# zhoujun-7/VPHO

Measured on AMD Instinct MI355X. Metric: eval images/sec (bs=64, sample_num=100, steps=50); MPJPE delta vs ref, higher is better.
Workload: dtype f32; 1 GPU; vpho_net.forward(mode=predict), README eval config (BASELINE.json configs[1]); per_gpu_batch=64, sample_num=100, sampling_steps=50, topk_hand=30, topk_obj=10, crop=256x256, pipeline_depth=3, parallelism=dp1, score_mfma=f32, conv_mfma=f32, winograd_3x3=True

## Files before the change

### include/vpho_hip.h

```cpp
#ifndef VPHO_HIP_H
#define VPHO_HIP_H

#if defined(__GNUC__) || defined(__clang__)
#define VPHO_API __attribute__((visibility("default")))
#else
#define VPHO_API
#endif

#ifdef __cplusplus
extern "C" {
#endif

VPHO_API const char* vpho_last_error(void);
VPHO_API int vpho_abi_version(void);

VPHO_API int vpho_prof_enable(int kernel_class, int on);
VPHO_API int vpho_prof_collect(int kernel_class, double* total_ms, long long* launches, double* total_flops, double* total_bytes);

typedef struct {
    const float* x; const float* w; const float* bias;
    const float* in_scale; const float* in_shift;
    const float* res; float* y;
    int N, H, W, Cin, x_ld;
    int Cout, KH, KW, stride, pad_y, pad_x, OH, OW;
    long long y_sn, y_sy, y_sx;
    long long r_sn, r_sy, r_sx;
    float in_slope, out_slope;
    int w_ld, splits;
    long long x_split, w_split, y_split;
    const float* gate;
    float gate_slope;
    const int* row_map;
    const int* row_count;
    int rows_hint;
    int rows_scatter;
    const void* w_planes;
    int plane_terms;
    const float* res_up;
    int ru_H, ru_W, ru_ld;
    const float* x2;
    int Cin2, x2_ld, stride2, H2, W2;
    int groups;
    long long x_group, w_group, bias_group, y_group, res_group, x2_group, pre_group, ru_group;
    float* stats;
    int* stats_rows;
    int stats_cap;
    const float* bn_x; const float* bn_mean; const float* bn_invstd; const float* bn_gamma; const float* bn_beta;
} vpho_conv_desc;
VPHO_API int vpho_conv2d_nhwc_f32(const vpho_conv_desc* d, void* stream);
VPHO_API int vpho_conv3x3_winograd_nhwc_f32(const float* x, const float* u, const float* bias, int N, int H, int W, int Cin, int x_ld, int Cout,
                                   float out_slope, float* y, int y_ld, void* stream);
VPHO_API int vpho_conv3x3_winograd_grouped_nhwc_f32(const float* x, long long x_group, const float* u, const float* bias, int groups, int N, int H, int W,
                                           int Cin, int x_ld, int Cout, float out_slope, float* y, int y_ld, void* stream);
VPHO_API int vpho_winograd_window_tiles_i32(const int* wins, int N, int* tile_base, void* stream);
VPHO_API int vpho_conv3x3_winograd_scatter_nhwc_f32(const float* x, const float* u, const float* bias, int N, int H, int W, int Cin, int x_ld, int Cout,
                                           float out_slope, const int* wins, const int* tile_base, float* y, int y_ld, void* stream);
VPHO_API int vpho_winograd_weights_f32(const float* w_packed, int Cout, int Cin, int for_input_gradient, float* u, void* stream);
VPHO_API int vpho_winograd_weights_multi_f32(const void* segments, int n_segments, long long total_blocks, void* stream);
VPHO_API int vpho_conv3x3_winograd_gate_nhwc_f32(const float* x, const float* u, const float* gate, float gate_slope, int N, int H, int W, int Cin,
                                        int x_ld, int Cout, float* y, int y_ld, void* stream);
VPHO_API int vpho_conv3x3_winograd_stats_nhwc_f32(const float* x, const float* u, const float* bias, int N, int H, int W, int Cin, int x_ld, int Cout,
                                         float out_slope, float* y, int y_ld, float* stats, int stats_cap, int* stats_rows, const float* bn_x,
                                         const float* bn_mean, const float* bn_invstd, const float* bn_gamma, const float* bn_beta,
                                         float gate_slope, void* stream);
VPHO_API int vpho_conv3x3_winograd_rows_nhwc_f32(const float* x, const float* u, const float* bias, int N, int H, int W, int Cin, int x_ld, int Cout,
                                        float out_slope, const int* wins, const int* tile_base, int tiles_hint, float* y_rows, int y_ld,
                                        void* stream);

typedef struct {
    int D, Dp, nheads;
    const float *t_W, *t_w, *t_b, *pe0_w, *pe0_b, *pe2_w, *pe2_b, *w1_t, *w1_p, *w1_f, *b1, *w2, *b2;
    const void* w1_p_split;
    int split_terms;
} vpho_score_weights;

VPHO_API long long vpho_score_workspace_bytes(const vpho_score_weights* w, int bs, int S);

VPHO_API int vpho_score_eval(const vpho_score_weights* w, const float* feat_img, int bs, int S, const float* x, float t,
                    float* out, void* workspace, long long workspace_bytes, void* stream);

typedef struct {
    int nfev;
    int n_accepted, n_rejected;
    int nan_count;
    int status;
    int n_log;
} vpho_ode_stats;

VPHO_API int vpho_ode_sample(const vpho_score_weights* w, const float* feat_img, int bs, int S, const float* init_x,
                    double T0, double eps, int num_steps, double rtol, double atol,
                    void* xs_out, int xs_is_f64, void* x_out, int x_is_f64,
                    void* workspace, long long workspace_bytes,
                    vpho_ode_stats* stats_host, double* step_log_host, int step_log_cap, void* stream);

VPHO_API int vpho_nchw_to_nhwc_f32(const float* x, int N, int C, int H, int W, float* y, int ldy, void* stream);
VPHO_API int vpho_nhwc_to_nchw_f32(const float* x, int N, int H, int W, int C, int ldx, float* y, void* stream);
VPHO_API int vpho_maxpool_nhwc_f32(const float* x, int N, int H, int W, int C, int k, int stride, int pad, float* y, void* stream);
VPHO_API int vpho_resize_bilinear_nhwc_f32(const float* x, int N, int H, int W, int C, int ldx, int OH, int OW,
                                  float* y, int ldy, int c_off, int accumulate, void* stream);
VPHO_API int vpho_roi_align_nhwc_f32(const float* feat, int N, int H, int W, int C, const float* boxes, float spatial_scale,
                            int out_size, const unsigned char* flip_w, float* out, int ldo, int c_off, void* stream);
VPHO_API int vpho_roi_windows_i32(const float* boxes_a, const float* boxes_b, int N, int H, int W, float spatial_scale, int dilate,
                         int* wins, int* row_map, int* row_count, void* stream);
VPHO_API int vpho_resize_bilinear_rows_nhwc_f32(const float* x, int N, int H, int W, int C, int ldx, int OH, int OW, float* y, int ldy, int c_off,
                                       int accumulate, const int* row_map, const int* row_count, int rows_hint, void* stream);
VPHO_API int vpho_roi_align_window_nhwc_f32(const float* feat_rows, const int* wins, int N, int H, int W, int C, const float* boxes,
                                   float spatial_scale, int out_size, const unsigned char* flip_w, float* out, int ldo, int c_off, int rows_hint,
                                   void* stream);
VPHO_API int vpho_roi_align_window_dual_nhwc_f32(const float* feat_rows, const int* wins, int N, int H, int W, int C, const float* boxes,
                                        float spatial_scale, int out_size, const unsigned char* flip_w, float* out, int ldo, int c_off,
                                        const unsigned char* flip_w2, float* out2, int ldo2, int c_off2, int rows_hint, void* stream);
VPHO_API int vpho_align_heatmap_nhwc_f32(const float* hm, int N, int size, int C, const float* bbox, const float* bbox_rect,
                                const unsigned char* flip_w, float* out, void* stream);
VPHO_API int vpho_linear_acc64_f32(const float* x, int rows, int cin, int ld_x, const float* w, const float* bias, int cout, float out_slope,
                          float* y, int ld_y, void* stream);
VPHO_API int vpho_nerf_embed_f32(const float* g, int N, const unsigned char* flip_x, float* out, void* stream);
VPHO_API int vpho_cross_tokens_f32(const float* proj_hand, const float* proj_obj, const float* grav_emb, const float* pe,
                          int bs, float* out, void* stream);
VPHO_API int vpho_mha_f32(const float* qkv, int S, int B, int E, int nhead, float* out, void* stream);
VPHO_API int vpho_mha_dropout_f32(const float* qkv, int S, int B, int E, int nhead, const float* drop_mask, float* out, void* stream);
VPHO_API int vpho_add_layernorm_f32(const float* x, const float* r, const float* gamma, const float* beta, long long rows, int E,
                           float eps, float* out, void* stream);
VPHO_API int vpho_force_local_f32(const float* scale, int ld_scale, const float* logits, int ld_logits, const float* anchor,
                         float friction, long long rows, int group, int group_stride, int off_scale, int off_logits,
                         float* out, void* stream);
VPHO_API int vpho_rot6d_to_axis_angle_f32(const float* x, long long rows, int rot_per_row, int ldx, float* out, int ldo, void* stream);
VPHO_API int vpho_append_betas_f32(const float* betas, long long rows, long long rows_per_image, float* out, int ldo, void* stream);

typedef struct {
    const float *v_template;
    const float *shapedirs;
    const float *posedirs_t;
    const float *J_regressor;
    const float *weights;
    const float *tip_posedirs_t;
    const float *posedirs_mfma;
} vpho_mano_tables;
VPHO_API int vpho_mano_shape_f32(const vpho_mano_tables* t, const float* betas, int n_img, float* v_shaped, float* J, void* stream);
VPHO_API int vpho_mano_fk_f32(const vpho_mano_tables* t, const float* pose, int ld_pose, long long n_hands, int hands_per_image,
                     const float* v_shaped, const float* J, const unsigned char* ho3d_per_image,
                     float* verts, float* joints, void* stream);

typedef struct { const float* kpt; const float* vert; const float* com; int n_kpt, n_vert, n_obj; } vpho_obj_tables;
typedef struct { const int* face_idx; const float* anchor_weight; const float* vert2joint; const int* skeleton; } vpho_anchor_tables;

VPHO_API int vpho_hand_candidates_f32(const float* diff_pose, int ld_diff, const float* reg_pose, int bs, int S, float* pose, void* stream);
VPHO_API int vpho_hand_heat_f32(const float* joints, const float* root, const float* Kmat, const float* bbox, const float* heatmap,
                       int bs, int C, int J, int H, int W, const int* observe_host, int n_obs, float* out, void* stream);
VPHO_API int vpho_hand_fuse_level_f32(const float* hv, int n_obs, float* pose, int bs, int C, int k, int level,
                             float* val, int* idx, float* topk_pose, float* score_out, void* stream);
VPHO_API int vpho_topk_f32(const float* scores, int rows_outer, int n, int F, int k, float* val, int* idx, void* stream);
VPHO_API int vpho_topk_weights_f32(const float* val, int rows, int k, float* w, void* stream);
VPHO_API int vpho_obj_heat_score(const double* pose, int n, const double* transl_override, const float* root, const vpho_obj_tables* t,
                        const int* obj_id, const unsigned char* is_right, const float* Kmat, const float* bbox,
                        const float* heatmap, int bs, int H, int W, float* score, void* stream);
VPHO_API int vpho_obj_cross_candidates(const double* pose, int n, const int* transl_idx, const int* rot_idx, int bs, int ko, double* cand, void* stream);
VPHO_API int vpho_obj_physics_score(const double* cand, int n, const float* root, const vpho_obj_tables* t, const int* obj_id,
                           const unsigned char* is_right, const float* force_point, const float* force_global, int bs,
                           float* score, void* stream);
VPHO_API int vpho_obj_fuse_f64(const double* pose, int n, const int* idx_a, const float* w_a, const int* idx_b, const float* w_b,
                      const unsigned char* pick_b, int bs, int k, double* fused, void* stream);
VPHO_API int vpho_obj_verts_f32(const double* pose, const float* root, const vpho_obj_tables* t, const int* obj_id,
                       const unsigned char* is_right, int bs, float* out, void* stream);
VPHO_API int vpho_force_anchor_f32(const vpho_anchor_tables* t, const float* verts, const float* root, const float* force_local,
                          long long n_hands, int hands_per_image, float* force_point, float* force_global, void* stream);
VPHO_API int vpho_hand_phys_candidates_f32(const float* agg_pose, int ld_agg, const float* betas, const float* topk_pose, int bs, int k,
                                  float* out, void* stream);
VPHO_API int vpho_hand_phys_score_f32(const float* force_point, const float* force_global, const float* obj_vert, int n_vert,
                             int bs, int n_cand, float* finger_score, void* stream);
VPHO_API int vpho_hand_phys_fuse_f32(const float* cand, int n_cand, const int* idx, int bs, int k, float* out, void* stream);

VPHO_API int vpho_heatmap_peak_f32(const float* heatmap, long long n_maps, int H, int W, float* peak, int* ind, void* stream);
VPHO_API int vpho_hand_pt2d_score_f32(const float* joints, const float* root, const float* Kmat, const float* bbox, const float* peak,
                             int bs, int C, int per_joint, float* score, void* stream);
VPHO_API int vpho_obj_pt2d_score(const double* pose, int n, const float* root, const vpho_obj_tables* t, const int* obj_id,
                        const unsigned char* is_right, const float* Kmat, const float* bbox, const float* peak, int bs,
                        float* score, void* stream);
VPHO_API int vpho_hand_pose_fuse_f32(const float* pose, int ld_pose, int C, const int* idx, const float* w, int bs, int n, float* fused,
                            void* stream);
VPHO_API int vpho_hand_joint_gather_mean_f32(const float* joints, const int* idx, int bs, int C, int k, float* fused, void* stream);
// ... 198 lines not shown
```

### vpho_amd/model/engine.py

```python
import os

import torch

from .. import ops
from ..configs.args import cfg, AGGREGATION_MODES_HAND, AGGREGATION_MODES_OBJ
from . import pack as P

MANO_JOINT_LEVEL = {0: [0], 1: [1, 5, 9, 13, 17], 2: [2, 6, 10, 14, 18], 3: [3, 7, 11, 15, 19], 4: [4, 8, 12, 16, 20]}
PHY_TOPK = 5
DEFAULT_MODE = 'heatmap_cascade'


def _signature(model):
    import itertools
    v = p = 0
    for t in itertools.chain(model.parameters(), model.buffers()):
        v += t._version
        p ^= t.data_ptr()
    return v, p, str(next(model.parameters()).device)


def _stack2(a, b):
    if torch.is_tensor(a):
        return torch.stack([a, b]).contiguous()
# ... 25 lines not shown
            out = []
            for i in range(blocks):
                p = f'{fe}.{name}.0.{i}'
                blk = dict(c1=fold(p + '.conv1', p + '.bn1'), c2=fold(p + '.conv2', p + '.bn2'),
                           c3=fold(p + '.conv3', p + '.bn3'), stride=stride if i == 0 else 1, down=None)
                if (p + '.downsample.0.weight') in sd:
                    blk['down'] = fold(p + '.downsample.0', p + '.downsample.1')
                    blk['c3_down'] = (torch.cat([blk['c3'][0], blk['down'][0]], 1).contiguous(), (blk['c3'][1] + blk['down'][1]).contiguous())
                out.append(blk)
            return out

        self.layers = dict(layer1_h=res_layer('layer1_h', 3, 1), layer2_h=res_layer('layer2_h', 4, 2),
                           layer3_h=res_layer('layer3_h', 6, 2), layer4_h=res_layer('layer4_h', 3, 2),
                           layer2_o=res_layer('layer2_o', 4, 2), layer3_o=res_layer('layer3_o', 6, 2))
        self.fpn = {k: fold(f'{fe}.{k}') for k in ('toplayer_h', 'toplayer_o', 'smooth3_h', 'smooth3_o', 'latlayer1_h',
                                                   'latlayer2_h', 'latlayer3_h', 'latlayer1_o', 'latlayer2_o', 'latlayer3_o')}

        def hm_head(p):
            s, t = P.bn_affine(sd, p + '.deconv_layers.1')
            wd = sd[p + '.deconv_layers.0.weight'] * s[None, :, None, None]
            phases = {k: (d(w), py, px) for k, (w, py, px) in P.pack_deconv4x4s2(wd).items()}
            return dict(c0=fold(p + '.conv_layers.0'), c1=fold(p + '.conv_layers.1', p + '.conv_layers.2'), deconv=phases,
                        deconv_b=d(t), final=fold(p + '.final_layer'))

        self.hm = dict(hand=hm_head('head_hm_hand'), obj=hm_head('head_hm_obj'))

        def encoder(p, cin):
            cin_pad = (cin + 3) // 4 * 4
            blocks = []
            for i in range(8):
                q = f'{p}.reg.{i}'
                s, t = P.bn_affine(sd, q + '.bn')
                blocks.append(dict(pre=(d(s), d(t)), c1=fold(q + '.conv1', q + '.bn1'), c2=fold(q + '.conv2', q + '.bn2'), c3=fold(q + '.conv3')))
            return dict(project=fold(p + '.project', cin_pad=cin_pad), blocks=blocks, cin_pad=cin_pad)

        self.enc = dict(hand=encoder('encoder_hand', 277), obj=encoder('encoder_obj', 283))

        self.grouped = os.environ.get('VPHO_GROUPED', '1') != '0'
        self.head64 = os.environ.get('VPHO_HEAD_F64', '1') != '0'
        if self.grouped:
            L, F = self.layers, self.fpn
            self.g_layers = dict(layer2=_stack2(L['layer2_h'], L['layer2_o']), layer3=_stack2(L['layer3_h'], L['layer3_o']))
            self.g_fpn = {k: _stack2(F[k + '_h'], F[k + '_o']) for k in ('toplayer', 'latlayer1', 'latlayer2')}
            self.g_hm = _stack2(*({k: v for k, v in self.hm[s].items() if k != 'final'} for s in ('hand', 'obj')))
            self.g_enc = _stack2(encoder('encoder_hand', 283), self.enc['obj'])

        lin = lambda p: (d(sd[p + '.weight']), d(sd[p + '.bias']))
        self.head_mano = dict(l0=lin('head_mano.base_layer.0'), l2=lin('head_mano.base_layer.2'), pose=lin('head_mano.fc_pose'),
                              shape=lin('head_mano.fc_shape'))

        def cross(p):
            a = p + '.attn.layers.0'
            return dict(proj_hand=fold(p + '.proj_hand'), proj_obj=fold(p + '.proj_obj'),
                        grav=(d(torch.nn.functional.pad(sd[p + '.gravity_proj.weight'], (0, 1))), d(sd[p + '.gravity_proj.bias'])),
                        pe=d(sd[p + '.pose_embedder.pe'][:, 0, :]),
                        in_proj=(d(sd[a + '.self_attn.in_proj_weight']), d(sd[a + '.self_attn.in_proj_bias'])),
                        out_proj=lin(a + '.self_attn.out_proj'), l1=lin(a + '.linear1'), l2=lin(a + '.linear2'),
                        n1=lin(a + '.norm1'), n2=lin(a + '.norm2'))

        self.cross = dict(hand=cross('cross_hand'), obj=cross('cross_obj'))
        self.phys = dict(s0=lin('head_physics.fc_scale.0'), s2=lin('head_physics.fc_scale.2'), w0=lin('head_physics.fc_weight.0'),
                         w2=lin('head_physics.fc_weight.2'), anchor=d(sd['head_physics.anchor']))

        self.score_hand = ops.ScoreNet(sd, 'denoiser_hand', dev)
        self.score_obj = ops.ScoreNet(sd, 'denoiser_obj', dev)
        mano = dict(v_template=sd['head_mano.mano_layer.th_v_template'][0], shapedirs=sd['head_mano.mano_layer.th_shapedirs'],
                    posedirs=sd['head_mano.mano_layer.th_posedirs'], J_regressor=sd['head_mano.mano_layer.th_J_regressor'],
                    weights=sd['head_mano.mano_layer.th_weights'])
        self.mano = ops.Mano(mano, dev)
        names = model.head_obj.names
        ycb = {n: dict(kpt3d=sd[f'head_obj.point_{n}'], verts_sampled=sd[f'head_obj.vert_{n}'], CoM=sd[f'head_obj.CoM_{n}'][0]) for n in names}
        self.agg = ops.Aggregation(dict(ycb=ycb, anchor=model.assets['anchor']), model.anchor_skeleton, dev)
        self.last_info = {}
        self._obj_stream = None
        self._pin = {}
        from concurrent.futures import ThreadPoolExecutor
        self._obj_worker = ThreadPoolExecutor(max_workers=1, thread_name_prefix='vpho-obj-sampler')
        self.use_graphs = os.environ.get('VPHO_GRAPHS', '1') != '0'
        self.roi_window = os.environ.get('VPHO_ROI_WINDOW', '1') != '0'
        self.feature_streams = int(os.environ.get('VPHO_FEATURE_STREAMS', '1'))
        self.fpn_fuse = os.environ.get('VPHO_FPN_FUSE', '1') != '0'
        self.down_fuse = os.environ.get('VPHO_DOWN_FUSE', '1') != '0'
        self.winograd = os.environ.get('VPHO_WINOGRAD', '1') != '0'
        self.conv_terms = {'f32': 0, 'bf16x6': 6, 'bf16x9': 9}[os.environ.get('VPHO_CONV_MFMA', 'f32')]
        self.serial_samplers = False
        self.device_prior = os.environ.get('VPHO_DEVICE_PRIOR', '0') == '1'
        self.keep_states = False
        self._feat_side = None
        self._two_streams = False
        from .graphs import GraphedCall
        self._features_graph = GraphedCall(self.features, dev)
        self._aggregate_graph = GraphedCall(self._aggregate_from_tensors, dev)

    def stale(self, model):
        return _signature(model) != self.sig

    def _bottleneck(self, x, b, out=None, groups=1, x_shared=False):
        y = ops.conv2d_nhwc(x, *b['c1'], out_slope=0.01, groups=groups, x_shared=x_shared)
        if b['stride'] == 1:
            y = ops.conv3x3(y, *b['c2'], out_slope=0.01, winograd=self.winograd, groups=groups)
        else:
            y = ops.conv2d_nhwc(y, *b['c2'], kh=3, kw=3, stride=b['stride'], pad=1, out_slope=0.01, groups=groups)
        if b['down'] is not None and self.down_fuse and x.shape[-1] % 32 == 0 and y.shape[-1] % 32 == 0:
            return ops.conv2d_nhwc(y, *b['c3_down'], x2=x, stride2=b['stride'], out_slope=0.01, out=out, groups=groups, x2_shared=x_shared)
        r = x if b['down'] is None else ops.conv2d_nhwc(x, *b['down'], stride=b['stride'], groups=groups, x_shared=x_shared)
        return ops.conv2d_nhwc(y, *b['c3'], res=r, out_slope=0.01, out=out, groups=groups)

    def _layer(self, x, blocks, out=None, groups=1, x_shared=False):
        for i, b in enumerate(blocks):
            x = self._bottleneck(x, b, out if i == len(blocks) - 1 else None, groups, x_shared and i == 0)
        return x

    def _side(self):
        import contextlib
        if not self._two_streams:
            return contextlib.nullcontext()
        if self._feat_side is None:
            self._feat_side = torch.cuda.Stream(self.dev)
        self._feat_side.wait_stream(torch.cuda.current_stream())
        return torch.cuda.stream(self._feat_side)

    def _join(self):
        if self._two_streams:
            torch.cuda.current_stream().wait_stream(self._feat_side)

    def _stem(self, rgb):
        x = ops.nchw_to_nhwc(rgb, 4)
        c1 = ops.maxpool_nhwc(ops.conv2d_nhwc(x, *self.stem, kh=7, kw=7, stride=2, pad=3, out_slope=0.01), 3, 2, 1)
        return self._layer(c1, self.layers['layer1_h'])

    def _lateral(self, c, wb, p, rows=None, groups=1):
        if self.fpn_fuse:
            return ops.conv2d_nhwc(c, *wb, rows=rows, rows_scatter=rows is not None, res_up=p, groups=groups)
        q = ops.conv2d_nhwc(c, *wb, rows=rows, rows_scatter=rows is not None, groups=groups)
        return ops.resize_bilinear_nhwc(p, q.shape[1], q.shape[2], out=q, accumulate=True, rows=rows)

    def _top_down(self, fpn, sfx, c5, c4, c3, groups=1):
        p = ops.conv2d_nhwc(c5, *fpn['toplayer' + sfx], groups=groups)
        p = self._lateral(c4, fpn['latlayer1' + sfx], p, groups=groups)
        return self._lateral(c3, fpn['latlayer2' + sfx], p, groups=groups)

    def _fpn_out(self, br, c2, p3, win, halo):
        p = self._lateral(c2, self.fpn[f'latlayer3_{br}'], p3, rows=halo)
        return ops.conv3x3(p, *self.fpn[f'smooth3_{br}'], winograd=self.winograd, rows=win)

    def _hm_up(self, x, h, groups=1):
        y = ops.conv3x3(x, *h['c0'], winograd=self.winograd, groups=groups)
        y = ops.conv3x3(y, *h['c1'], winograd=self.winograd, groups=groups)
        N, H, W, _ = y.shape
        co = h['deconv_b'].shape[-1]
        up = torch.empty((N, 2 * H, 2 * W, co), device=y.device)
        for (py, px), (w, pady, padx) in h['deconv'].items():
            ops.conv2d_nhwc(y, w, h['deconv_b'], kh=2, kw=2, pad_y=pady, pad_x=padx, out_hw=(H, W), out_slope=0.0, groups=groups,
                            out_view=(up, 4 * H * W * co, 4 * W * co, 2 * co, (py * 2 * W + px) * co))
        return up

    def _encoder(self, x, e, groups=1):
        x = ops.conv2d_nhwc(x, *e['project'], groups=groups)
        stages = []
        for i, b in enumerate(e['blocks']):
            y = ops.conv2d_nhwc(x, *b['c1'], in_scale=b['pre'][0], in_shift=b['pre'][1], in_slope=0.01, out_slope=0.01, groups=groups)
            y = ops.conv3x3(y, *b['c2'], out_slope=0.01, winograd=self.winograd, groups=groups)
            x = ops.conv2d_nhwc(y, *b['c3'], res=x, groups=groups)
            if i % 2 == 1:
                x = ops.maxpool_nhwc(x, 2, 2, 0)
                stages.append(x)
        N = x.shape[0]
        return ops.nhwc_to_nchw(x).view(N, -1), stages

    def _cross(self, c, st_h, st_o, grav, flip_u8):
        bs = st_h.shape[0]
        ph = ops.conv3x3(st_h, *c['proj_hand'], winograd=self.winograd)
        po = ops.conv3x3(st_o, *c['proj_obj'], winograd=self.winograd)
        ge = ops.linear(ops.nerf_embed(grav, flip_u8), *c['grav'])
        x = ops.cross_tokens(ph, po, ge, c['pe']).view(bs * 65, 512)
        qkv = ops.linear(x, *c['in_proj'])
        o = ops.linear(ops.mha(qkv, bs, 65, 512, 2).view(bs * 65, 512), *c['out_proj'])
        x = ops.add_layernorm(x, o, *c['n1'])
        ff = ops.linear(ops.linear(x, *c['l1'], out_slope=0.0), *c['l2'])
        return ops.add_layernorm(x, ff, *c['n2'])

    def features(self, data):
        grouped = self.grouped and self.conv_terms == 0
        self._two_streams = self.feature_streams >= 2 and not grouped
        with ops.conv_split(self.conv_terms):
            rgb = data['rgb'].float().contiguous()
            bs = rgb.shape[0]
            f32 = lambda k: data[k].float().contiguous()
            left_u8 = (~data['is_right'].bool()).to(torch.uint8).contiguous()
            bb_h, bb_o, bb_hr, bb_or = f32('bbox_hand'), f32('bbox_obj'), f32('bbox_hand_rect'), f32('bbox_obj_rect')
            win_h = win_o = halo_h = halo_o = None
            if self.roi_window:
                fh, fw = rgb.shape[2] // 4, rgb.shape[3] // 4
                win_h = ops.roi_windows(bb_h, bb_hr, bs, fh, fw, 0.25)
                win_o = ops.roi_windows(bb_or, None, bs, fh, fw, 0.25)
                halo_h, halo_o = ops.roi_windows(bb_h, bb_hr, bs, fh, fw, 0.25, dilate=1), ops.roi_windows(bb_or, None, bs, fh, fw, 0.25, dilate=1)
            grav = f32('gravity').view(bs, 3)
            twin = self._twin_grouped if grouped else self._twin_per_branch
            (hand_feat, obj_feat, hf_hr, in_h, in_o, hm_hand, hm_obj, hand_heatmap, obj_heatmap, enc_h, enc_o, st_h, st_o) = twin(
                rgb, (bb_h, bb_o, bb_hr, bb_or), (win_h, win_o, halo_h, halo_o), left_u8)
            with self._side():
                tok_o = self._cross(self.cross['obj'], st_h, st_o, grav, left_u8)
            hmn = self.head_mano
            a64 = self.head64
            h = ops.linear(ops.linear(enc_h, *hmn['l0'], out_slope=0.01, acc64=a64), *hmn['l2'], out_slope=0.01, acc64=a64)
            pose = ops.rot6d_to_axis_angle(ops.linear(h, *hmn['pose'], acc64=a64), 16)
            shape = ops.linear(h, *hmn['shape'], acc64=a64)
            ctx = self.mano.shape(shape)
            ho3d = data['is_ho3d'].to(torch.uint8).contiguous() if 'is_ho3d' in data else None
            reg_vert, reg_joint = self.mano.fk(pose, ctx, 1, True, ho3d)
            tok_h = self._cross(self.cross['hand'], st_h, st_o, grav, left_u8)
# ... 178 lines not shown
        return A.obj_fuse(obj_pose, idx, None), info

    def aggregate(self, f, data, final58, obj_pose, S, k_hand, k_obj, oid=None, mode_hand=DEFAULT_MODE, mode_obj=DEFAULT_MODE, weighted=True):
        self._check_modes(f, S, k_hand, k_obj, mode_hand, mode_obj)
        A, M = self.agg, self.mano
        bs = obj_pose.shape[0]
        if mode_hand != DEFAULT_MODE or mode_obj != DEFAULT_MODE:
            f32 = lambda k: data[k].float().contiguous()
            Kmat = f32('cam_intr_crop_flip').view(bs, 9)
            res, dbg = {}, {}
            if mode_hand == DEFAULT_MODE or mode_obj == DEFAULT_MODE:
                res, dbg = self.aggregate(f, data, final58, obj_pose, S, k_hand, k_obj, oid=oid)
            dbg.update(mode_hand=mode_hand, mode_obj=mode_obj)
            if mode_hand != DEFAULT_MODE:
                (mano, vert, joint), dbg['hand_mode'] = self._aggregate_hand_mode(mode_hand, f, final58, f32('root_joint_flip'), Kmat, f32('bbox_hand'),
                                                                                  S, k_hand, weighted)
                res.update(hand_agg_mano=mano, hand_agg_vert=vert, hand_agg_joint=joint)
            if mode_obj != DEFAULT_MODE:
                oid = A.obj_ids(data['obj_name']) if oid is None else oid
                isr = data['is_right'].to(torch.uint8).contiguous()
                res['obj_agg_6d'], dbg['obj_mode'] = self._aggregate_obj_mode(mode_obj, f, obj_pose, f32('root_joint'), oid, isr, Kmat,
                                                                              f32('bbox_obj_rect'), k_obj)
            return res, dbg
        f32 = lambda k: data[k].float().contiguous()
        root_flip, root, Kmat = f32('root_joint_flip'), f32('root_joint'), f32('cam_intr_crop_flip').view(bs, 9)
        bb_h, bb_or = f32('bbox_hand'), f32('bbox_obj_rect')
        isr = data['is_right'].to(torch.uint8).contiguous()
        ungrasp = (~data['is_grasped'].bool()).to(torch.uint8).contiguous()
        oid = A.obj_ids(data['obj_name']) if oid is None else oid
        ctx = f['mano_ctx']
        dbg = dict(hand_topk=[], hand_val=[])
        if self.keep_states:
            dbg['cascade_state'], dbg['hand_score'] = [], []
        pose = A.hand_candidates(final58, f['mano_pose'], bs, S)
        tp = None
        for level in range(4):
            observe = [j for l in range(level + 1, 5) for j in MANO_JOINT_LEVEL[l]]
            if self.keep_states:
                dbg['cascade_state'].append(pose.clone())
            _, joints = M.fk(pose.view(-1, 48), ctx, 2 * S, False)
            hv = A.hand_heat(joints.view(bs, 2 * S, 21, 3), root_flip, Kmat, bb_h, f['hand_heatmap'], observe)
            if self.keep_states:
                val, idx, tp, sc = A.hand_fuse_level(hv, pose, k_hand, level, want_topk_pose=(level == 3), want_scores=True)
                dbg['hand_score'].append(sc)
            else:
                val, idx, tp = A.hand_fuse_level(hv, pose, k_hand, level, want_topk_pose=(level == 3))
            dbg['hand_topk'].append(idx)
            dbg['hand_val'].append(val)
        fused_rows = pose.view(bs, 2 * S * 48)
        agg_vert, _ = M.fk(fused_rows, ctx, 1, True)
        fpnt, fglob = A.force_anchor(agg_vert, root_flip, f['force_local'], 1)
        hm_o = f['obj_heatmap']
        sc = A.obj_heat_score(obj_pose, root, oid, isr, Kmat, bb_or, hm_o)
        tv, ti = A.topk(sc, k_obj)
        transl = A.obj_fuse(obj_pose, ti.view(bs, -1), A.topk_weights(tv).view(bs, -1))[:, 6:].contiguous()
        sc2 = A.obj_heat_score(obj_pose, root, oid, isr, Kmat, bb_or, hm_o, transl_override=transl)
        _, ri = A.topk(sc2, k_obj)
        cand = A.obj_cross(obj_pose, ti.view(bs, -1), ri.view(bs, -1))
        ps = A.obj_physics_score(cand, root, oid, isr, fpnt, fglob)
        _, pi = A.topk(ps, PHY_TOPK)
        hs = A.obj_heat_score(cand, root, oid, isr, Kmat, bb_or, hm_o)
        hval, hi = A.topk(hs, PHY_TOPK)
        obj_fused = A.obj_fuse(cand, pi.view(bs, -1), None, hi.view(bs, -1), A.topk_weights(hval).view(bs, -1), ungrasp)
        obj_vert = A.obj_verts(obj_fused, root, oid, isr)
        cand58 = A.hand_phys_candidates(fused_rows, f['mano_shape'], tp)
        n_c = cand58.shape[1]
        cverts, _ = M.fk(cand58.view(-1, 58), ctx, n_c, True)
        fp2, fg2 = A.force_anchor(cverts, root_flip, f['force_local'], n_c)
        fs = A.hand_phys_score(fp2, fg2, obj_vert, bs, n_c)
        _, fidx = A.topk(fs, PHY_TOPK, 5)
        out58 = A.hand_phys_fuse(cand58, fidx)
        out_vert, out_joint = M.fk(out58, ctx, 1, True)
        dbg.update(transl_topk=ti, rot_topk=ri, phys_topk=pi, heat_topk=hi, phys_score=ps, transl_score=sc, rot_score=sc2, heat_score=hs, hand_phys_topk=fidx, hand_phys_score=fs, cand58=cand58, cand_vert=cverts, cand_force_point=fp2, cand_force_global=fg2,
                   cascade_pose=fused_rows[:, :48], force_point=fpnt, force_global=fglob, obj_vert=obj_vert, pose6d_candidate=cand, transl=transl)
        return dict(obj_agg_6d=obj_fused, hand_agg_mano=out58, hand_agg_vert=out_vert, hand_agg_joint=out_joint), dbg

    @torch.no_grad()
    def predict(self, data, noise_hand=None, noise_obj=None, mode_hand=None, mode_obj=None):
        S, T0, steps = cfg.sample_num, cfg.sample_T0, cfg.sampling_steps
        modes = dict(mode_hand=cfg.aggregation_mode_hand if mode_hand is None else mode_hand,
                     mode_obj=cfg.aggregation_mode_obj if mode_obj is None else mode_obj, weighted=bool(cfg.do_weighted_average))
        with torch.cuda.device(self.dev):
            if self.use_graphs:
                f = self._features_graph({k: v for k, v in data.items() if torch.is_tensor(v)}, (cfg.roi_size, cfg.heatmap_size, self.conv_terms, self.roi_window, self.feature_streams, self.winograd, self.fpn_fuse, self.down_fuse))
                keep = lambda t: t.clone()
            else:
                f = self.features(data)
                keep = lambda t: t
            bs = f['mano_pose'].shape[0]
            sig = 0.01 * (50 / 0.01) ** T0
            init_h = self._prior(bs * S, 96) if noise_hand is None else noise_hand.float()
            init_o = self._prior(bs * S, 9) if noise_obj is None else noise_obj.float()
            init_h, init_o = init_h.to(self.dev, non_blocking=True) * sig, init_o.to(self.dev, non_blocking=True) * sig
            out = dict(reg_hand_vert=keep(f['reg_hand_vert']), reg_hand_joint=keep(f['reg_hand_joint']), hand_heatmap=keep(f['hand_heatmap']),
                       obj_heatmap=keep(f['obj_heatmap']), force_local=keep(f['force_local']))
            main = torch.cuda.current_stream()
            if self._obj_stream is None:
                self._obj_stream = torch.cuda.Stream(device=self.dev)
            obj_stream = self._obj_stream
            obj_stream.wait_stream(main)

            def run_obj():
                with torch.cuda.device(self.dev), torch.cuda.stream(obj_stream):
                    return self.score_obj.sample(f['encoding_obj'], init_o, S, T0, steps, xs_f64=True, x_f64=True)

            concurrent = os.environ.get('VPHO_SERIAL_SAMPLERS', '0') != '1' and not self.serial_samplers
            fut = self._obj_worker.submit(run_obj) if concurrent else None
            xs_h, x_h, st_h = self.score_hand.sample(f['encoding_hand'], init_h, S, T0, steps, xs_f64=False, x_f64=False)
            inproc = torch.empty((bs * S * steps, 58), device=self.dev)
            ops.rot6d_to_axis_angle(xs_h.view(bs * S * steps, 96), 16, out=inproc)
            ops.append_betas(f['mano_shape'], inproc, S * steps)
            final = torch.empty((bs * S, 58), device=self.dev)
            ops.rot6d_to_axis_angle(x_h, 16, out=final)
            ops.append_betas(f['mano_shape'], final, S)
            out['diff_inprocess_hand_mano'] = inproc.view(bs, S, steps, 58)
            out['diff_final_hand_mano'] = final.view(bs, S, 58)
            ctx = f['mano_ctx']
            viz = inproc.view(bs * S, steps, 58)[0, ::10].contiguous()
            vv, vj = self.mano.fk(viz, ctx, viz.shape[0], True)
            out['diff_inprocess_hand_vert'], out['diff_inprocess_hand_joint'] = vv, vj
            fv, fj = self.mano.fk(final, ctx, S, True)
            out['diff_final_hand_vert'] = fv.view(bs, S, 778, 3)
            out['diff_final_hand_joint'] = fj.view(bs, S, 21, 3)
            xs_o, x_o, st_o = fut.result() if fut is not None else run_obj()
            main.wait_stream(obj_stream)
            for t in (xs_o, x_o):
                t.record_stream(main)
            out['diff_inprocess_obj_6d'] = xs_o.view(bs, S, steps, 9)
            out['diff_final_obj_6d'] = x_o.view(bs, S, 9)
            for name, st in (('hand', st_h), ('obj', st_o)):
                if st['nan_count']:
                    print("\033[31mWarning: NaN detected in score evaluation. \033[0m")
            x_o9 = out['diff_final_obj_6d']
            if self.use_graphs:
                agg, dbg = self.aggregate_graphed(f, data, final, x_o9, S, cfg.topk_hand, cfg.topk_obj, **modes)
            else:
                agg, dbg = self.aggregate(f, data, final, x_o9, S, cfg.topk_hand, cfg.topk_obj, **modes)
            out['agg_obj_6d'] = keep(agg['obj_agg_6d'])
            out['agg_hand_mano'] = keep(agg['hand_agg_mano'])
            out['agg_hand_vert'] = keep(agg['hand_agg_vert'])
            out['agg_hand_joint'] = keep(agg['hand_agg_joint'])
            self.last_info = dict(features=f, hand_ode=st_h, obj_ode=st_o, agg=dbg, hand_x6d=x_h)
        return out
```

### vpho_amd/ops.py

```python
import ctypes as C
import os

import torch

_HERE = os.path.dirname(os.path.abspath(__file__))
LIB_PATH = os.environ.get('VPHO_HIP_LIB') or os.path.join(_HERE, 'libvpho_hip.so')

if not os.path.exists(LIB_PATH):
    raise ImportError(f'{LIB_PATH} is missing: build the HIP extension first (python -m vpho_amd.build or '
                      f'__graft_entry__.build()); vpho_amd has no CPU fallback')
lib = C.CDLL(LIB_PATH)
lib.vpho_last_error.restype = C.c_char_p
lib.vpho_abi_version.restype = C.c_int
ABI_VERSION = 13
if lib.vpho_abi_version() != ABI_VERSION:
    raise ImportError(f'{LIB_PATH} implements ABI version {lib.vpho_abi_version()}, this binding expects {ABI_VERSION}: rebuild the '
                      f'extension (python -m vpho_amd.build --force)')
lib.vpho_obj_metrics_workspace_bytes.restype = C.c_longlong
lib.vpho_obj_metrics_multi_workspace_bytes.restype = C.c_longlong
lib.vpho_bn_workspace_bytes.restype = C.c_longlong
lib.vpho_conv2d_wgrad_workspace_bytes.restype = C.c_longlong
lib.vpho_mha_bwd_workspace_bytes.restype = C.c_longlong
lib.vpho_grad_sqnorm_workspace_bytes.restype = C.c_longlong
lib.vpho_infer_record_bytes.restype = C.c_longlong
# ... 458 lines not shown
        need = lib.vpho_score_workspace_bytes(C.byref(self.c), bs, S)
        if self._ws is None or self._ws.numel() < need:
            self._ws = torch.empty(need, dtype=torch.uint8, device=self.device)
        return self._ws

    def score(self, feat_img, x, t, S):
        bs = feat_img.shape[0]
        ws = self.workspace(bs, S)
        out = torch.empty((bs * S, self.D), device=self.device, dtype=torch.float32)
        _check(lib.vpho_score_eval(C.byref(self.c), _ptr(feat_img, torch.float32), bs, S, _ptr(x, torch.float32), float(t),
                                   _ptr(out), _ptr(ws), ws.numel(), _stream()))
        return out

    def sample(self, feat_img, init_x, S, T0, num_steps, xs_f64, x_f64=True, eps=1e-5, rtol=3e-3, atol=3e-4, log_cap=4096):
        bs = feat_img.shape[0]
        R = bs * S
        assert init_x.shape == (R, self.D)
        ws = self.workspace(bs, S)
        xs = torch.empty((R, num_steps, self.D), device=self.device, dtype=torch.float64 if xs_f64 else torch.float32)
        x = torch.empty((R, self.D), device=self.device, dtype=torch.float64 if x_f64 else torch.float32)
        st = OdeStats()
        log = (C.c_double * (4 * log_cap))()
        _check(lib.vpho_ode_sample(C.byref(self.c), _ptr(feat_img, torch.float32), bs, S, _ptr(init_x, torch.float32),
                                   float(T0), float(eps), int(num_steps), float(rtol), float(atol), _ptr(xs),
                                   1 if xs_f64 else 0, _ptr(x), 1 if x_f64 else 0, _ptr(ws), ws.numel(), C.byref(st), log, log_cap,
                                   _stream()))
        n = min(st.n_log, log_cap)
        steps = [(log[4 * i], log[4 * i + 1], log[4 * i + 2], bool(log[4 * i + 3])) for i in range(n)]
        return xs, x, dict(nfev=st.nfev, n_accepted=st.n_accepted, n_rejected=st.n_rejected, nan_count=st.nan_count,
                           steps=steps)


def _i32(t):
    return _ptr(t, torch.int32)


def _u8(t):
    return None if t is None else _ptr(t, torch.uint8)


def _f32(t):
    return None if t is None else _ptr(t, torch.float32)


def _f64(t):
    return None if t is None else _ptr(t, torch.float64)


def _call(name, *args):
    _check(getattr(lib, name)(*args, _stream()))


def _new(shape, like, dtype=torch.float32):
    return torch.empty(shape, device=like.device, dtype=dtype)


LL, I, F = C.c_longlong, C.c_int, C.c_float


def nchw_to_nhwc(x, ld=None):
    N, Cc, H, W = x.shape
    ld = Cc if ld is None else ld
    y = _new((N, H, W, ld), x)
    _call('vpho_nchw_to_nhwc_f32', _f32(x), I(N), I(Cc), I(H), I(W), _f32(y), I(ld))
    return y


def nhwc_to_nchw(x, channels=None):
    N, H, W, ld = x.shape
    Cc = ld if channels is None else channels
    y = _new((N, Cc, H, W), x)
    _call('vpho_nhwc_to_nchw_f32', _f32(x), I(N), I(H), I(W), I(Cc), I(ld), _f32(y))
    return y


def maxpool_nhwc(x, k, stride, pad):
    N, H, W, Cc = x.shape
    OH, OW = (H + 2 * pad - k) // stride + 1, (W + 2 * pad - k) // stride + 1
    y = _new((N, OH, OW, Cc), x)
    _call('vpho_maxpool_nhwc_f32', _f32(x), I(N), I(H), I(W), I(Cc), I(k), I(stride), I(pad), _f32(y))
    return y


def resize_bilinear_nhwc(x, OH, OW, out=None, c_off=0, accumulate=False, channels=None, rows=None):
    N, H, W, ldx = x.shape
    Cc = ldx if channels is None else channels
    if out is None:
        out = _new((N, OH, OW, Cc), x)
    assert out.shape[:3] == (N, OH, OW)
    if rows is not None:
        assert rows.shape == (N, OH, OW)
        _call('vpho_resize_bilinear_rows_nhwc_f32', _f32(x), I(N), I(H), I(W), I(Cc), I(ldx), I(OH), I(OW), _f32(out), I(out.shape[-1]),
              I(c_off), I(1 if accumulate else 0), _ptr(rows.row_map, torch.int32), _ptr(rows.count, torch.int32),
              I(int(rows.count.item()) if _prof_on else 0))
        return out
    _call('vpho_resize_bilinear_nhwc_f32', _f32(x), I(N), I(H), I(W), I(Cc), I(ldx), I(OH), I(OW), _f32(out), I(out.shape[-1]),
          I(c_off), I(1 if accumulate else 0))
    return out


class RoiWindows:
    def __init__(self, wins, row_map, count, shape):
        self.wins, self.row_map, self.count, self.shape = wins, row_map, count, shape
        self._tiles = None

    def tiles(self):
        if self._tiles is None:
            self._tiles = torch.empty((self.shape[0] + 1,), device=self.wins.device, dtype=torch.int32)
            _call('vpho_winograd_window_tiles_i32', _i32(self.wins), I(self.shape[0]), _i32(self._tiles))
        return self._tiles

    def to_map(self, rows):
        n = int(self.count.item())
        N, H, W = self.shape
        idx = self.row_map[:n].long()
        full = torch.zeros((N * H * W, rows.shape[-1]), device=rows.device, dtype=rows.dtype)
        full[idx] = rows[:n]
        mask = torch.zeros((N * H * W,), device=rows.device, dtype=torch.bool)
        mask[idx] = True
        return full.view(N, H, W, -1), mask.view(N, H, W)


def roi_windows(boxes_a, boxes_b, N, H, W, spatial_scale, dilate=0):
    dev = boxes_a.device
    wins = torch.empty((N, 5), device=dev, dtype=torch.int32)
    row_map = torch.empty((N * H * W,), device=dev, dtype=torch.int32)
    count = torch.empty((1,), device=dev, dtype=torch.int32)
    _call('vpho_roi_windows_i32', _f32(boxes_a), _f32(boxes_b), I(N), I(H), I(W), F(spatial_scale), I(dilate), _ptr(wins, torch.int32),
          _ptr(row_map, torch.int32), _ptr(count, torch.int32))
    return RoiWindows(wins, row_map, count, (N, H, W))


def roi_align_nhwc(feat, boxes, out_size, spatial_scale, flip_w=None, out=None, c_off=0, win=None):
    if win is not None:
        N, H, W = win.shape
        Cc = feat.shape[-1]
        if out is None:
            out = _new((N, out_size, out_size, Cc), feat)
        _call('vpho_roi_align_window_nhwc_f32', _f32(feat), _ptr(win.wins, torch.int32), I(N), I(H), I(W), I(Cc), _f32(boxes),
              F(spatial_scale), I(out_size), _u8(flip_w), _f32(out), I(out.shape[-1]), I(c_off), I(int(win.count.item()) if _prof_on else 0))
        return out
    N, H, W, Cc = feat.shape
    if out is None:
        out = _new((N, out_size, out_size, Cc), feat)
    _call('vpho_roi_align_nhwc_f32', _f32(feat), I(N), I(H), I(W), I(Cc), _f32(boxes), F(spatial_scale), I(out_size), _u8(flip_w),
          _f32(out), I(out.shape[-1]), I(c_off))
    return out


def roi_align_dual_nhwc(feat, boxes, out_size, spatial_scale, win, out2, flip_w2=None, c_off2=0, out=None):
    N, H, W = win.shape
    Cc = feat.shape[-1]
    if out is None:
        out = _new((N, out_size, out_size, Cc), feat)
    assert out.shape == (N, out_size, out_size, Cc) and out.is_contiguous()
    _call('vpho_roi_align_window_dual_nhwc_f32', _f32(feat), _ptr(win.wins, torch.int32), I(N), I(H), I(W), I(Cc), _f32(boxes),
          F(spatial_scale), I(out_size), _u8(None), _f32(out), I(Cc), I(0), _u8(flip_w2), _f32(out2), I(out2.shape[-1]), I(c_off2),
          I(int(win.count.item()) if _prof_on else 0))
    return out


def align_heatmap_nhwc(hm, bbox, bbox_rect, flip_w=None):
    N, S, _, Cc = hm.shape
    out = torch.empty_like(hm)
    _call('vpho_align_heatmap_nhwc_f32', _f32(hm), I(N), I(S), I(Cc), _f32(bbox), _f32(bbox_rect), _u8(flip_w), _f32(out))
    return out
# ... 1281 lines not shown
```

Before: 2233 images/s.

## Fuse stem 7x7 conv, LeakyReLU and maxpool into one MFMA kernel

Replaces the three-launch ResNet stem (NCHW->NHWC transpose, 7x7 stride-2 conv, 3x3 maxpool) with a single HIP kernel. It reads the NCHW RGB patch straight into LDS with buffer-load-to-LDS, runs the conv as f32 MFMA with the taps paired and double-buffered, applies bias and LeakyReLU, then max-pools from LDS before writing. This removes the full-resolution conv output round trip through global memory and two extra launches. The cost is a halo recompute per tile plus a large, hand-scheduled kernel that must match the old path numerically.

```diff
diff --git a/include/vpho_hip.h b/include/vpho_hip.h
--- a/include/vpho_hip.h
+++ b/include/vpho_hip.h
@@ -96,6 +96,7 @@
 VPHO_API int vpho_nchw_to_nhwc_f32(const float* x, int N, int C, int H, int W, float* y, int ldy, void* stream);
 VPHO_API int vpho_nhwc_to_nchw_f32(const float* x, int N, int H, int W, int C, int ldx, float* y, void* stream);
 VPHO_API int vpho_maxpool_nhwc_f32(const float* x, int N, int H, int W, int C, int k, int stride, int pad, float* y, void* stream);
+VPHO_API int vpho_stem7x7_pool_f32(const float* rgb, const float* w, const float* bias, int N, int H, int W, float out_slope, float* y, void* stream);
 VPHO_API int vpho_resize_bilinear_nhwc_f32(const float* x, int N, int H, int W, int C, int ldx, int OH, int OW,
                                   float* y, int ldy, int c_off, int accumulate, void* stream);
 VPHO_API int vpho_roi_align_nhwc_f32(const float* feat, int N, int H, int W, int C, const float* boxes, float spatial_scale,
diff --git a/vpho_amd/csrc/stem.hip b/vpho_amd/csrc/stem.hip
--- /dev/null
+++ b/vpho_amd/csrc/stem.hip
@@ -0,0 +1,197 @@
+#include "common.h"
+#include "../../include/vpho_hip.h"
+#include <algorithm>
+#include <cmath>
+
+namespace {
+
+constexpr int TPH = 8, TPW = 16;
+constexpr int CH = 2 * TPH + 1, CW = 2 * TPW + 1;
+constexpr int CPIX = CH * CW;
+constexpr int MT = (CPIX + 31) / 32;
+constexpr int PR = 2 * (CH - 1) + 7, PC = 2 * (CW - 1) + 7;
+constexpr int PLD = 72;
+constexpr int NT = 256, NWAVES = 4;
+constexpr int FILLS = (3 * PR * PLD + 64 * NWAVES - 1) / (64 * NWAVES);
+constexpr int PATCH_F = FILLS * NWAVES * 64;
+constexpr int SCH = 16;
+constexpr int SLICE_F = MT * 32 * SCH;
+constexpr int STAGE_F = SLICE_F > PATCH_F ? SLICE_F : PATCH_F;
+constexpr int NP = 25;
+constexpr int W_F = NP * 3 * 128;
+constexpr int MPW = MT / 2;
+static_assert(MT % 2 == 0 && (STAGE_F + W_F) * 4 <= 80 * 1024, "two workgroups per CU");
+
+struct StemGeo {
+    const float* x; const float* w; const float* bias; float* y;
+    int N, H, W, OH, OW, PH, PW;
+    int tiles_y, tiles_x, ntiles;
+    float slope;
+};
+
+__global__ __launch_bounds__(NT, 2) void stem7x7_pool_kernel(const StemGeo g) {
+    __shared__ __attribute__((aligned(1024))) float smem[STAGE_F + W_F];
+    float* const patch = smem;
+    float* const S = smem;
+    float* const Wl = smem + STAGE_F;
+
+    const int tid = threadIdx.x, lane = tid & 63, wave = __builtin_amdgcn_readfirstlane(tid >> 6);
+    const int li = lane & 31, lh = lane >> 5;
+    const int nh = wave & 1, mg = wave >> 1;
+
+    for (int i = tid; i < 64 * 49; i += NT) {
+        const int co = i / 49, tap = i - 49 * co;
+        const f32x4 v = *reinterpret_cast<const f32x4*>(g.w + 4 * i);
+        float* const d = Wl + (tap >> 1) * 3 * 128 + (co >> 5) * 64 + (tap & 1) * 32 + (co & 31);
+        d[0] = v[0]; d[128] = v[1]; d[256] = v[2];
+    }
+    if (tid < 3 * 64) Wl[((NP - 1) * 3 + (tid >> 6)) * 128 + ((tid >> 5) & 1) * 64 + 32 + (tid & 31)] = 0.f;
+    const float bv = g.bias ? g.bias[nh * 32 + li] : 0.f;
+
+    int a_base[MPW];
+#pragma unroll
+    for (int i = 0; i < MPW; ++i) {
+        int m = (mg * MPW + i) * 32 + li;
+        if (m >= CPIX) m = 0;
+        const int cy = m / CW, cx = m - cy * CW;
+        a_base[i] = 2 * cy * PLD + 2 * cx + lh;
+    }
+    const int wrap = lh * (PLD - 7);
+
+    const __amdgpu_buffer_rsrc_t xr = __builtin_amdgcn_make_buffer_rsrc(const_cast<float*>(g.x), 0, 0xFFFFFFF0u, 0x00020000);
+    typedef __attribute__((address_space(3))) void* lds_ptr;
+
+    for (int tile = blockIdx.x; tile < g.ntiles; tile += gridDim.x) {
+        const int tx = tile % g.tiles_x, t2 = tile / g.tiles_x;
+        const int ty = t2 % g.tiles_y, n = t2 / g.tiles_y;
+        const int py0 = ty * TPH, px0 = tx * TPW;
+        const int cy0 = 2 * py0 - 1, cx0 = 2 * px0 - 1;
+        const int iy0 = 2 * cy0 - 3, ix0 = 2 * cx0 - 3;
+
+#pragma unroll 3
+        for (int j = 0; j < FILLS; ++j) {
+            const int i = (wave * FILLS + j) * 64 + lane;
+            const int row = i / PLD, col = i - row * PLD;
+            const int c = row / PR, r = row - c * PR;
+            const int iy = iy0 + r, ix = ix0 + col;
+            const bool ok = c < 3 && (unsigned)iy < (unsigned)g.H && (unsigned)ix < (unsigned)g.W;
+            const unsigned off = ok ? ((unsigned)((n * 3 + c) * g.H + iy) * (unsigned)g.W + (unsigned)ix) * 4u : 0xFFFFFFFFu;
+            __builtin_amdgcn_raw_ptr_buffer_load_lds(xr, (lds_ptr)(patch + (wave * FILLS + j) * 64), 4, (int)off, 0, 0, 0);
+        }
+        VPHO_SYNC_LDS_DMA();
+
+        f32x16 acc[MPW];
+#pragma unroll
+        for (int i = 0; i < MPW; ++i)
+#pragma unroll
+            for (int e = 0; e < 16; ++e) acc[i][e] = 0.f;
+        const float* const Bw = Wl + nh * 64 + lane;
+        auto load = [&](int s, float (&a)[MPW], float& b) {
+            const int P = s / 3, c = s - 3 * P;
+            const int t = 2 * P, ky = t / 7, kx = t - 7 * ky;
+            const bool row_end = kx == 6 && P != NP - 1;
+            const int off = (c * PR + ky) * PLD + kx;
+            b = Bw[s * 128];
+#pragma unroll
+            for (int i = 0; i < MPW; ++i) {
+                a[i] = patch[a_base[i] + (row_end ? wrap : 0) + off];
+                if (P == NP - 1) a[i] = lh ? 0.f : a[i];
+            }
+        };
+        auto mm = [&](const float (&a)[MPW], const float b) {
+#pragma unroll
+            for (int i = 0; i < MPW; ++i) acc[i] = __builtin_amdgcn_mfma_f32_32x32x2f32(a[i], b, acc[i], 0, 0, 0);
+        };
+        float a0[MPW], a1[MPW], b0, b1;
+        static_assert((3 * NP) % 2 == 1, "the step loop below ends on the even buffer");
+        load(0, a0, b0);
+#pragma unroll
+        for (int s = 0; s + 2 < 3 * NP; s += 2) {
+            load(s + 1, a1, b1);
+            __builtin_amdgcn_sched_barrier(0);
+            mm(a0, b0);
+            __builtin_amdgcn_sched_barrier(0);
+            load(s + 2, a0, b0);
+            __builtin_amdgcn_sched_barrier(0);
+            mm(a1, b1);
+            __builtin_amdgcn_sched_barrier(0);
+        }
+        mm(a0, b0);
+        __syncthreads();
+
+#pragma unroll
+        for (int i = 0; i < MPW; ++i)
+#pragma unroll
+            for (int e = 0; e < 16; ++e) {
+                const float v = acc[i][e] + bv + 0.f;
+                acc[i][e] = v > 0.f ? v : v * g.slope;
+            }
+#pragma unroll
+        for (int r = 0; r < 64 / SCH; ++r) {
+            if (nh == (r >> 1) && (li >> 4) == (r & 1)) {
+#pragma unroll
+                for (int i = 0; i < MPW; ++i)
+#pragma unroll
+                    for (int e = 0; e < 16; ++e) {
+                        const int m = (mg * MPW + i) * 32 + (e & 3) + 8 * (e >> 2) + 4 * lh;
+                        S[m * SCH + (li & 15)] = acc[i][e];
+                    }
+            }
+            __syncthreads();
+#pragma unroll
+            for (int it = 0; it < TPH * TPW * (SCH / 4) / NT; ++it) {
+                const int idx = tid + it * NT;
+                const int p = idx >> 2, q = idx & 3;
+                const int ply = p / TPW, plx = p - ply * TPW;
+                const int gy = py0 + ply, gx = px0 + plx;
+                if (gy >= g.PH || gx >= g.PW) continue;
+                const float* const sp = S + (2 * ply * CW + 2 * plx) * SCH + 4 * q;
+                f32x4 v[9];
+#pragma unroll
+                for (int w = 0; w < 9; ++w) v[w] = *reinterpret_cast<const f32x4*>(sp + ((w / 3) * CW + w % 3) * SCH);
+                f32x4 mx = {-INFINITY, -INFINITY, -INFINITY, -INFINITY};
+#pragma unroll
+                for (int w = 0; w < 9; ++w) {
+                    const bool in = (unsigned)(cy0 + 2 * ply + w / 3) < (unsigned)g.OH && (unsigned)(cx0 + 2 * plx + w % 3) < (unsigned)g.OW;
+#pragma unroll
+                    for (int k = 0; k < 4; ++k) mx[k] = fmaxf(mx[k], in ? v[w][k] : -INFINITY);
+                }
+                *reinterpret_cast<f32x4*>(g.y + (((long long)n * g.PH + gy) * g.PW + gx) * 64 + SCH * r + 4 * q) = mx;
+            }
+            __syncthreads();
+        }
+    }
+}
+
+}
+
+extern "C" int vpho_stem7x7_pool_f32(const float* rgb, const float* w, const float* bias, int N, int H, int W, float out_slope, float* y, void* stream) {
+    VPHO_REQUIRE(rgb && w && y && N > 0 && H > 0 && W > 0, "vpho_stem7x7_pool_f32: bad argument");
+    VPHO_REQUIRE(((uintptr_t)y & 15) == 0 && ((uintptr_t)w & 15) == 0 && ((uintptr_t)rgb & 3) == 0, "vpho_stem7x7_pool_f32: w and y must be 16-byte aligned");
+    StemGeo g;
+    g.x = rgb; g.w = w; g.bias = bias; g.y = y;
+    g.N = N; g.H = H; g.W = W;
+    g.OH = (H + 6 - 7) / 2 + 1; g.OW = (W + 6 - 7) / 2 + 1;
+    g.PH = (g.OH + 2 - 3) / 2 + 1; g.PW = (g.OW + 2 - 3) / 2 + 1;
+    VPHO_REQUIRE(12.0 * N * H * (double)W < 3.9e9, "vpho_stem7x7_pool_f32: the input must stay below 3.9 GB");
+    g.tiles_y = (g.PH + TPH - 1) / TPH; g.tiles_x = (g.PW + TPW - 1) / TPW;
+    const long long ntiles = (long long)N * g.tiles_y * g.tiles_x;
+    VPHO_REQUIRE(ntiles < (1ll << 31), "vpho_stem7x7_pool_f32: too many tiles");
+    g.ntiles = (int)ntiles;
+    g.slope = out_slope;
+    static int slots_of[64] = {0};
+    int dev = 0;
+    VPHO_HIP(hipGetDevice(&dev));
+    int& slots = slots_of[dev & 63];
+    if (!slots) {
+        hipDeviceProp_t prop;
+        VPHO_HIP(hipGetDeviceProperties(&prop, dev));
+        slots = 2 * prop.multiProcessorCount;
+    }
+    hipStream_t s = (hipStream_t)stream;
+    const double flops = 2.0 * N * g.OH * g.OW * 64.0 * 147.0;
+    const double bytes = 4.0 * (3.0 * N * H * W + 64.0 * 196.0 + 64.0 + 64.0 * N * g.PH * g.PW);
+    vpho::ProfScope prof(vpho::PROF_CONV128x64, s, flops, bytes);
+    hipLaunchKernelGGL(stem7x7_pool_kernel, dim3(std::min(g.ntiles, slots)), dim3(NT), 0, s, g);
+    return vpho::check_launch("stem7x7_pool_kernel");
+}
diff --git a/vpho_amd/model/engine.py b/vpho_amd/model/engine.py
--- a/vpho_amd/model/engine.py
+++ b/vpho_amd/model/engine.py
@@ -131,6 +131,7 @@
         self.fpn_fuse = os.environ.get('VPHO_FPN_FUSE', '1') != '0'
         self.down_fuse = os.environ.get('VPHO_DOWN_FUSE', '1') != '0'
         self.winograd = os.environ.get('VPHO_WINOGRAD', '1') != '0'
+        self.stem_fused = os.environ.get('VPHO_STEM_FUSED', '1') != '0'
         self.conv_terms = {'f32': 0, 'bf16x6': 6, 'bf16x9': 9}[os.environ.get('VPHO_CONV_MFMA', 'f32')]
         self.serial_samplers = False
         self.device_prior = os.environ.get('VPHO_DEVICE_PRIOR', '0') == '1'
@@ -174,8 +175,12 @@
             torch.cuda.current_stream().wait_stream(self._feat_side)
 
     def _stem(self, rgb):
-        x = ops.nchw_to_nhwc(rgb, 4)
-        c1 = ops.maxpool_nhwc(ops.conv2d_nhwc(x, *self.stem, kh=7, kw=7, stride=2, pad=3, out_slope=0.01), 3, 2, 1)
+        w = self.stem[0]
+        if self.stem_fused and rgb.dtype == torch.float32 and rgb.dim() == 4 and rgb.shape[1] == 3 and tuple(w.shape) == (64, 7 * 7 * 4):
+            c1 = ops.stem7x7_pool(rgb, *self.stem, out_slope=0.01)
+        else:
+            x = ops.nchw_to_nhwc(rgb, 4)
+            c1 = ops.maxpool_nhwc(ops.conv2d_nhwc(x, *self.stem, kh=7, kw=7, stride=2, pad=3, out_slope=0.01), 3, 2, 1)
         return self._layer(c1, self.layers['layer1_h'])
 
     def _lateral(self, c, wb, p, rows=None, groups=1):
@@ -520,7 +525,7 @@
                      mode_obj=cfg.aggregation_mode_obj if mode_obj is None else mode_obj, weighted=bool(cfg.do_weighted_average))
         with torch.cuda.device(self.dev):
             if self.use_graphs:
-                f = self._features_graph({k: v for k, v in data.items() if torch.is_tensor(v)}, (cfg.roi_size, cfg.heatmap_size, self.conv_terms, self.roi_window, self.feature_streams, self.winograd, self.fpn_fuse, self.down_fuse))
+                f = self._features_graph({k: v for k, v in data.items() if torch.is_tensor(v)}, (cfg.roi_size, cfg.heatmap_size, self.conv_terms, self.roi_window, self.feature_streams, self.winograd, self.fpn_fuse, self.down_fuse, self.stem_fused))
                 keep = lambda t: t.clone()
             else:
                 f = self.features(data)
diff --git a/vpho_amd/ops.py b/vpho_amd/ops.py
--- a/vpho_amd/ops.py
+++ b/vpho_amd/ops.py
@@ -564,6 +564,15 @@
     return y
 
 
+def stem7x7_pool(rgb, w, bias=None, out_slope=1.0):
+    N, Cc, H, W = rgb.shape
+    assert Cc == 3 and tuple(w.shape) == (64, 196) and (bias is None or tuple(bias.shape) == (64,)), (rgb.shape, w.shape)
+    OH, OW = (H - 1) // 2 + 1, (W - 1) // 2 + 1
+    y = _new((N, (OH - 1) // 2 + 1, (OW - 1) // 2 + 1, 64), rgb)
+    _call('vpho_stem7x7_pool_f32', _f32(rgb), _f32(w), _f32(bias), I(N), I(H), I(W), F(out_slope), _f32(y))
+    return y
+
+
 def resize_bilinear_nhwc(x, OH, OW, out=None, c_off=0, accumulate=False, channels=None, rows=None):
     N, H, W, ldx = x.shape
     Cc = ldx if channels is None else channels
```

Measured after the change: 2252 images/s (median of 6 runs). No clear change (+0.8%).
